# lenskit/csr

Hardware: AMD Instinct MI355X
Metric: spmv_gflops (higher is better)
Workload: dtype f64

## Files before the change

### csr_amd/csrc/spmv.hip

```cpp
#include "spmv_plan.h"

#include <algorithm>
#include <ctime>

namespace csrk {
template <bool R32>
__device__ __forceinline__ double spmv_prod(double a, double x)
{
    const double t = a * x;
    return R32 ? (double)(float)t : t;
}

void free_spmv_plan(SpmvPlan *p) { delete p; }

void spmv_plan_bytes_by_part(const SpmvPlan *p, int64_t out[5])
{
    for (int i = 0; i < 5; i++) out[i] = 0;
    auto add = [&](int part, std::initializer_list<const DevBuf *> bufs) {
        for (const DevBuf *b : bufs) out[part] += (int64_t)b->bytes;
    };
    for (const AccPanel *ap : p->acc) add(0, {&ap->row_list, &ap->vals, &ap->idx, &ap->tile_row0, &ap->segs, &ap->wg_seg, &ap->partial, &ap->z});
    const Panel &t = p->tier1;
    add(1, {&t.row_list, &t.rp, &t.ci, &t.vs, &t.tile, &t.group, &t.carry_row, &t.carry_val, &t.y, &t.crp, &t.cidx});
    const LightStream *l = &p->ls;
    add(2, {&l->vals, &l->idx, &l->rowids, &l->tile_base, &l->carry_row, &l->carry_val});
    add(3, {&l->xg, &l->a_col, &l->a_dst, &l->blk_start, &l->round_start, &l->round_tile0, &l->wg_round0, &p->hot_slot, &p->hot_cols, &p->xh});
    add(4, {&p->tile_row, &p->carry_row, &p->carry_val, &p->rp_light, &p->cut_pos, &p->cut_cum, &p->tile_cut, &p->heavy_row, &p->seg_off,
            &p->seg_row, &p->seg_part, &p->xwide});
}

int64_t spmv_plan_bytes(const SpmvPlan *p)
{
    int64_t part[5];
    spmv_plan_bytes_by_part(p, part);
    return part[0] + part[1] + part[2] + part[3] + part[4];
}


template <int VT>
__device__ __forceinline__ void load_val_pair(const void *vs, int64_t k, bool two, double &v0, double &v1)
{
    if (VT == CSRK_VAL_F64) {
        const double *p = (const double *)vs + k;
        if (two) {
            f64x2_t t = __builtin_nontemporal_load((const F64x2 *)p);
            v0 = t.x;
            v1 = t.y;
        } else {
            v0 = *p;
            v1 = 0.0;
        }
    } else if (VT == CSRK_VAL_F32) {
        const float *p = (const float *)vs + k;
        if (two) {
// ... 349 lines not shown
        }
        __syncthreads();
        const int nlong = s_nlong;
        for (int q = wv; q < nlong; q += PT / WAVE) {
            int r = s_long[q];
            int s = r ? s_rend[r - 1] : 0;
            int e = s_rend[r];
            double acc = 0.0;
            for (int k = s + lane; k < e; k += WAVE) acc += s_prod[k];
            acc = wave_sum(acc);
            if (lane == 0) {
                if (r < nr) {
                    yp[i0 + r] = acc;
                } else {
                    *(pt.cslot >= 0 ? yp + pt.cslot : carry_val + t) = acc;
                }
            }
        }
        pt = nx;
    }
#undef PANEL_LOAD_TILE
}

typedef float f32x4_t __attribute__((ext_vector_type(4)));
template <class SV> struct AccVals;
template <> struct AccVals<double> {
    f64x2_t v[4];
    __device__ __forceinline__ void load(const double *tile, int lane)
    {
        const f64x2_t *vp = (const f64x2_t *)tile;
#pragma unroll
        for (int q = 0; q < 4; q++) v[q] = __builtin_nontemporal_load(vp + q * WAVE + lane);
    }
    __device__ __forceinline__ void get(double (&a)[ACC_K]) const
    {
#pragma unroll
        for (int q = 0; q < 4; q++) {
            a[2 * q] = v[q].x;
            a[2 * q + 1] = v[q].y;
        }
    }
};
template <> struct AccVals<float> {
    f32x4_t v[2];
    __device__ __forceinline__ void load(const float *tile, int lane)
    {
        const f32x4_t *vp = (const f32x4_t *)tile;
#pragma unroll
        for (int q = 0; q < 2; q++) v[q] = __builtin_nontemporal_load(vp + q * WAVE + lane);
    }
    __device__ __forceinline__ void get(double (&a)[ACC_K]) const
    {
#pragma unroll
        for (int q = 0; q < 2; q++) {
            a[4 * q] = (double)v[q].x;
            a[4 * q + 1] = (double)v[q].y;
            a[4 * q + 2] = (double)v[q].z;
            a[4 * q + 3] = (double)v[q].w;
        }
    }
};

template <int CB, int PT, bool R32 = false, class SV = double, class XT = double>
__global__ __launch_bounds__(PT) void spmv_acc_kernel(const SV *__restrict__ pvals, const uint16_t *__restrict__ pidx,
                                                     const int32_t *__restrict__ tile_row0,
                                                     const XT *__restrict__ x, int32_t ncols,
                                                     const AccSeg *__restrict__ segs, const int32_t *__restrict__ wg_seg,
                                                     int32_t H, double *__restrict__ partial)
{
    extern __shared__ __align__(16) unsigned char acc_smem[];
    double *s_x = (double *)acc_smem;
    double *s_acc = s_x + CB + 2;
    const int Hpad = (H + 1) & ~1;
    double *s_hval = s_acc + Hpad;
    int32_t *s_hrow = (int32_t *)(s_hval + ACC_SEG_TILES);
    constexpr int NW = PT / WAVE;
    const int tid = threadIdx.x, lane = tid & (WAVE - 1), wv = tid / WAVE;

    for (int h = tid; h < Hpad; h += PT) s_acc[h] = 0.0;
    if (tid < 2) s_x[CB + tid] = 0.0;
    const unsigned long long below = lane ? (~0ull >> (WAVE - lane)) : 0ull;
    const unsigned long long upto = below | (1ull << lane);

    int cur_blk = -1;
    const int sb = wg_seg[blockIdx.x], se = wg_seg[blockIdx.x + 1];
    for (int si = sb; si < se; si++) {
        const AccSeg sg = segs[si];
        if (sg.blk != cur_blk) {
            cur_blk = sg.blk;
            const int32_t w0 = sg.blk * CB;
            const int wlen = ncols - w0 < CB ? ncols - w0 : CB;
            if (wlen == CB) {
                constexpr int WL = CB / 2 / PT;
                f64x2_t v[WL];
#pragma unroll
                for (int u = 0; u < WL; u++) {
                    if (sizeof(XT) == 8) {
                        v[u] = *((const F64x2 *)(x + w0) + tid + u * PT);
                    } else {
                        const f32x2_t t = *((const F32x2 *)(x + w0) + tid + u * PT);
                        v[u].x = (double)t.x;
                        v[u].y = (double)t.y;
                    }
                }
#pragma unroll
                for (int u = 0; u < WL; u++) ((f64x2_t *)s_x)[tid + u * PT] = v[u];
            } else {
                for (int k = tid; k < wlen; k += PT) s_x[k] = (double)x[w0 + k];
            }
        }
        __syncthreads();

        const int nt = sg.ntiles;
        AccVals<SV> v, vn;
        u32x4_t ix, ixn;
        int32_t tr0 = 0, tr0n = 0;
        int t = wv;
        const int64_t pstep = (int64_t)gridDim.x;
        if (t < nt) {
            const u32x4_t *ip = (const u32x4_t *)(pidx + (sg.ptile0 + t * pstep) * ACC_TILE);
            v.load(pvals + (sg.ptile0 + t * pstep) * ACC_TILE, lane);
            ix = __builtin_nontemporal_load(ip + lane);
            tr0 = tile_row0[sg.tile0 + t];
        }
        for (; t < nt; t += NW) {
            const bool more = t + NW < nt;
            if (more) {
                const u32x4_t *ip = (const u32x4_t *)(pidx + (sg.ptile0 + (t + NW) * pstep) * ACC_TILE);
                vn.load(pvals + (sg.ptile0 + (t + NW) * pstep) * ACC_TILE, lane);
                ixn = __builtin_nontemporal_load(ip + lane);
                tr0n = tile_row0[sg.tile0 + t + NW];
            }
            const uint32_t e[ACC_K] = {ix.x & 0xffffu, ix.x >> 16, ix.y & 0xffffu, ix.y >> 16,
                                       ix.z & 0xffffu, ix.z >> 16, ix.w & 0xffffu, ix.w >> 16};
            double a[ACC_K];
            v.get(a);
            double xv[ACC_K];
#pragma unroll
            for (int j = 0; j < ACC_K; j++) xv[j] = s_x[e[j] & ACC_COL_MASK];
            int rw[ACC_K];
            {
                int lsum = 0;
#pragma unroll
                for (int j = 0; j < ACC_K; j++) lsum += (int)(e[j] >> ACC_ROW_SHIFT);
                int run = tr0 + wave_exscan_i32(lsum, lane);
#pragma unroll
                for (int j = 0; j < ACC_K; j++) {
                    run += (int)(e[j] >> ACC_ROW_SHIFT);
                    rw[j] = run;
                }
            }
            const int hr = rw[0];
            int cur = hr;
            double acc = 0.0, hs = 0.0;
            bool nb = false;
#pragma unroll
            for (int j = 0; j < ACC_K; j++) {
                const int r = rw[j];
                if (r != cur) {
                    if (!nb) {
                        hs = acc;
                        nb = true;
                    } else {
                        atomicAdd(&s_acc[cur], acc);
                    }
                    acc = 0.0;
                    cur = r;
                }
                if (R32) acc += spmv_prod<true>(a[j], xv[j]);
                else acc += a[j] * xv[j];
            }
            const int tr = cur;
            const double ts = acc;
            if (!nb) hs = acc;
            const int tr_prev = wave_up1_i32(tr, -1);
            const bool ne = lane > 0 && tr_prev != hr;
            const double T = wave_segscan(ts, nb || ne, lane);
            const double T_prev = wave_up1_f64(T, 0.0);
// ... 197 lines not shown
        tb = __builtin_amdgcn_readfirstlane(tile_base[t]);
    }
    for (int64_t R = R_begin; R < R_end; R += R_step) {
    if (RND) {
        __syncthreads();
#pragma unroll
        for (int q = 0; q < RQ; q++) ((f64x2_t *)s_rnd)[q * LS_THREADS + threadIdx.x] = rv[q];
        __syncthreads();
        if (R + R_step < R_end) round_request(R + R_step);
    }
    const int64_t rt1 = round_t1(R);
    for (t = round_t0(R) + wv; t < rt1; t += NW) {
        int64_t t_next = t + NW;
        if (t_next >= rt1) {
            t_next = t;
            if (R + R_step < R_end) {
                const int64_t tf = round_t0(R + R_step) + wv;
                if (tf < round_t1(R + R_step)) t_next = tf;
            }
        }
        uint32_t e[ACC_K];
        if constexpr (I24) {
            const uint32_t lo[4] = {ix[0].x, ix[0].y, ix[0].z, ix[0].w}, hi[2] = {ix[1].x, ix[1].y};
#pragma unroll
            for (int j = 0; j < ACC_K; j++)
                e[j] = __builtin_amdgcn_perm(hi[j >> 2], lo[j >> 1],
                                             0x0c000000u | ((4u + (j & 3)) << 16) | ((2u * (j & 1) + 1u) << 8) | (2u * (j & 1)));
        } else {
            const uint32_t w[ACC_K] = {ix[0].x, ix[0].y, ix[0].z, ix[0].w, ix[1].x, ix[1].y, ix[1].z, ix[1].w};
#pragma unroll
            for (int j = 0; j < ACC_K; j++) e[j] = w[j];
        }
        double a[ACC_K];
        v.get(a);
        double gv[ACC_K], lv[ACC_K];
        bool inl[ACC_K];
        if (RND) {
#pragma unroll
            for (int j = 0; j < ACC_K; j++) {
                const uint32_t c = e[j] & COL_MASK;
                const bool hot = (e[j] & HOT_BIT) != 0;
                inl[j] = c != PAD && (!hot || (int32_t)c < n_lds);
                gv[j] = 0.0;
                if (hot && (int32_t)c >= n_lds) gv[j] = xh[c];
            }
        } else {
#pragma unroll
            for (int j = 0; j < ACC_K; j++) {
                const uint32_t c = e[j] & LS_COL_MASK;
                const bool hot = (e[j] & LS_HOT_BIT) != 0;
                inl[j] = hot && (int32_t)c < n_lds;
                gv[j] = 0.0;
                const double *g = hot ? xh + c : x + c;
                if (!inl[j] && c != LS_PAD) gv[j] = *g;
            }
        }
        int32_t rid[LS_RID];
#pragma unroll
        for (int i = 0; i < LS_RID; i++) {
            const int run = tb - 1 + lane + i * WAVE;
            const int runc = run < 0 ? 0 : (run > n_runs - 1 ? n_runs - 1 : run);
            rid[i] = DENSE ? runc : rowids[runc];
        }
        asm volatile("" ::: "memory");
        {
            const int64_t tn = t_next;
            idx_request(ixn, tn);
// ... 238 lines not shown
                dn[q] = k < k1 ? __builtin_nontemporal_load(a_dst + k) : 0;
            }
        }
#pragma unroll
        for (int q = 0; q < LS_STAGE_IPT; q++)
            if (c[q] >= 0) xg[d[q]] = s_x[c[q]];
        if (kn < k1) {
#pragma unroll
            for (int q = 0; q < LS_STAGE_IPT; q++) c[q] = cn[q], d[q] = dn[q];
        }
    }
}

int spmv_kernel_attributes()
{
    for (const void *f : {(const void *)spmv_acc_kernel<ACC_CB, ACC_THREADS>, (const void *)spmv_lstream_kernel<LS_PLAIN>,
                          (const void *)spmv_lstream_kernel<LS_RND>, (const void *)spmv_lstream_kernel<LS_PLAIN, true>,
                          (const void *)spmv_lstream_kernel<LS_RND, true>, (const void *)spmv_acc_kernel<ACC_CB, ACC_THREADS, true>,
                          (const void *)spmv_lstream_kernel<LS_PLAIN, false, true>, (const void *)spmv_lstream_kernel<LS_RND, false, true>,
                          (const void *)spmv_lstream_kernel<LS_PLAIN, true, true>, (const void *)spmv_lstream_kernel<LS_RND, true, true>,
                          (const void *)spmv_acc_kernel<ACC_CB, ACC_THREADS, false, float>,
                          (const void *)spmv_acc_kernel<ACC_CB, ACC_THREADS, true, float>,
                          (const void *)spmv_lstream_kernel<LS_PLAIN, false, false, float>, (const void *)spmv_lstream_kernel<LS_RND, false, false, float>,
                          (const void *)spmv_lstream_kernel<LS_PLAIN, true, false, float>, (const void *)spmv_lstream_kernel<LS_RND, true, false, float>,
                          (const void *)spmv_lstream_kernel<LS_PLAIN, false, true, float>, (const void *)spmv_lstream_kernel<LS_RND, false, true, float>,
                          (const void *)spmv_lstream_kernel<LS_PLAIN, true, true, float>, (const void *)spmv_lstream_kernel<LS_RND, true, true, float>,
                          (const void *)spmv_lstream_kernel<LS_RND24>, (const void *)spmv_lstream_kernel<LS_RND24, true>,
                          (const void *)spmv_lstream_kernel<LS_RND24, false, true>, (const void *)spmv_lstream_kernel<LS_RND24, true, true>,
                          (const void *)spmv_lstream_kernel<LS_RND24, false, false, float>, (const void *)spmv_lstream_kernel<LS_RND24, true, false, float>,
                          (const void *)spmv_lstream_kernel<LS_RND24, false, true, float>, (const void *)spmv_lstream_kernel<LS_RND24, true, true, float>,
                          (const void *)spmv_acc_kernel<ACC_CB, ACC_THREADS, false, double, float>,
                          (const void *)spmv_acc_kernel<ACC_CB, ACC_THREADS, true, double, float>,
                          (const void *)spmv_acc_kernel<ACC_CB, ACC_THREADS, false, float, float>,
                          (const void *)spmv_acc_kernel<ACC_CB, ACC_THREADS, true, float, float>})
        CSRK_HIP(hipFuncSetAttribute(f, hipFuncAttributeMaxDynamicSharedMemorySize, (int)(160 * 1024)));
    CSRK_HIP(hipFuncSetAttribute((const void *)ls_stage_kernel<double>, hipFuncAttributeMaxDynamicSharedMemorySize, (int)(LS_STAGE_WMAX * 8)));
    CSRK_HIP(hipFuncSetAttribute((const void *)ls_stage_kernel<float>, hipFuncAttributeMaxDynamicSharedMemorySize, (int)(LS_STAGE_WMAX * 8)));
    return CSRK_OK;
}

static int get_plan_locked(Matrix *m, hipStream_t s, SpmvPlan **out, bool launching)
{
    if (launching) m->spmv_calls++;
    const char *env = getenv("CSRK_SPMV_HEAVY_SPLIT"), *env_hot = getenv("CSRK_SPMV_HOT"), *env_ls = getenv("CSRK_SPMV_STREAM");
    const bool eager = (env && env[0] == '1') || (env_hot && env_hot[0] == '1') || (env_ls && env_ls[0] == '1') || !launching;
    const bool want_split = eager || m->spmv_calls >= 2;
    if (m->spmv_plan && !m->spmv_plan->split_considered && want_split && m->spmv_plan->algo == CSRK_SPMV_MERGE &&
        !m->spmv_plan->profiling) {
        if (hipDeviceSynchronize() != hipSuccess) {
            set_error("device synchronisation failed: %s", hipGetErrorString(hipGetLastError()));
            return CSRK_ERR_HIP;
        }
        free_spmv_plan(m->spmv_plan);
        m->spmv_plan = nullptr;
    }
    if (!m->spmv_plan) {
        SpmvPlan *p = new (std::nothrow) SpmvPlan();
        CSRK_REQUIRE(p, "out of host memory");
        p->algo = m->spmv_algo == CSRK_SPMV_AUTO ? CSRK_SPMV_MERGE : m->spmv_algo;
        (void)s;
        int rc = build_spmv_plan(m, p, want_split);
        if (rc == CSRK_OK && hipDeviceSynchronize() != hipSuccess) {
            set_error("SpMV plan construction failed: %s", hipGetErrorString(hipGetLastError()));
            rc = CSRK_ERR_HIP;
        }
        if (rc != CSRK_OK) {
            delete p;
// ... 58 lines not shown
            J.row_list = rows;
            J.H = H;
            J.n_wg = n_wg;
            J.G = G;
            J.extra = extra;
            J.crp = crp;
            J.cidx = cidx;
            J.cval = cval;
            epi.j[epi.n++] = J;
            return CSRK_OK;
        };
        if (do_light && p->ls.on && p->ls.n_cold) {
            KernelTimer ks(p, s, 3);
            const unsigned gs = (unsigned)(ceil_div(p->ls.n_stage_blk, 8) * 8);
            ls_stage_kernel<XT><<<gs, LS_STAGE_THREADS, (size_t)p->ls.stage_w * 8, s>>>(
                d_x, m->ncols, p->ls.stage_w, p->ls.a_col.as<uint16_t>(), p->ls.a_dst.as<int32_t>(),
                p->ls.blk_start.as<int32_t>(), p->ls.n_stage_blk, p->ls.xg.as<double>());
            ks.stop();
            CSRK_LAUNCH_CHECK();
        }
        if (do_light && p->n_hot && !(p->ls.on && p->ls.n_cold)) {
            hot_pack_kernel<XT><<<(unsigned)ceil_div(p->n_hot, 256), 256, 0, s>>>(d_x, p->hot_cols.as<int32_t>(), p->n_hot,
                                                                            p->xh.as<double>());
            CSRK_LAUNCH_CHECK();
        }
        bool t0_rides = false;
        if (do_heavy && p->n_heavy && !p->acc.empty()) {
            KernelTimer kh(p, s, 1);
            for (AccPanel *ap : p->acc) {
                if (ap->f32)
                    spmv_acc_kernel<ACC_CB, ACC_THREADS, R32, float, XT><<<(unsigned)ap->n_wg, ACC_THREADS, ap->lds, s>>>(
                        ap->vals.as<float>(), ap->idx.as<uint16_t>(), ap->tile_row0.as<int32_t>(), d_x, m->ncols,
                        ap->segs.as<AccSeg>(), ap->wg_seg.as<int32_t>(), ap->nrow, ap->partial.as<double>());
                else
                    spmv_acc_kernel<ACC_CB, ACC_THREADS, R32, double, XT><<<(unsigned)ap->n_wg, ACC_THREADS, ap->lds, s>>>(
                        ap->vals.as<double>(), ap->idx.as<uint16_t>(), ap->tile_row0.as<int32_t>(), d_x, m->ncols,
                        ap->segs.as<AccSeg>(), ap->wg_seg.as<int32_t>(), ap->nrow, ap->partial.as<double>());
                CSRK_LAUNCH_CHECK();
            }
            kh.stop();
        }
        if (do_heavy && p->n_heavy && p->tier1.on) {
            Panel *pn = &p->tier1;
            KernelTimer kh(p, s, 2);
#define PANEL_ARGS(PP)                                                                                              \
    pn->rp.as<PP>(), pn->ci.as<int32_t>(), pn->vs.as<double>(), d_x, m->ncols, pn->y.as<double>(),                    \
        pn->tile.as<PanelTile>(), pn->group.as<PanelGroup>(), pn->rows, pn->carry_row.as<int32_t>(),                  \
        pn->carry_val.as<double>(), pn->nnz, pn->cb, rider
            PanelRider rider = {pn->groups, nullptr, nullptr, 0, 0};
            if (PANEL_T1 / WAVE == 4 && do_heavy && p->acc.size() == 1 && p->acc[0]->z.p) {
                AccPanel *ap = p->acc[0];
                rider.partial = ap->partial.as<double>();
                rider.z = ap->z.as<double>();
                rider.H = ap->nrow;
                rider.n_wg = ap->n_wg;
                t0_rides = true;
            }
            const unsigned grid = (unsigned)(pn->groups + (t0_rides ? ceil_div(rider.H, WAVE) : 0));
            if (pn->p64) spmv_panel_kernel<int64_t, PANEL_T1, R32, XT><<<grid, PANEL_T1, 0, s>>>(PANEL_ARGS(int64_t));
            else spmv_panel_kernel<int32_t, PANEL_T1, R32, XT><<<grid, PANEL_T1, 0, s>>>(PANEL_ARGS(int32_t));
#undef PANEL_ARGS
            kh.stop();
            CSRK_LAUNCH_CHECK();
        }
        if (do_light) {
#define MERGE_ARGS_LIGHT(CI)                                                                                        \
// ... 401 lines not shown
    for (int c = 0; c < 4; c++) mean_ms[c] = cnt[c] ? (float)(tot[c] / cnt[c]) : 0.f;
    p->ev_used = 0;
    return CSRK_OK;
}

int csrk_spmv_profile_end(csrk_handle_t h, int *n_records, float *mean_ms)
{
    float ms4[4] = {0.f, 0.f, 0.f, 0.f};
    CSRK_REQUIRE(n_records && mean_ms, "output is NULL");
    CSRK_TRY(csrk_spmv_profile_end4(h, n_records, ms4));
    for (int c = 0; c < 3; c++) mean_ms[c] = ms4[c];
    return CSRK_OK;
}

int csrk_spmv_plan_stats(csrk_handle_t h, int64_t *out, int n)
{
    Matrix *m = from_handle(h);
    if (!m) return CSRK_ERR_INVALID;
    CSRK_REQUIRE(out && n >= 0, "out is NULL");
    SpmvPlan *p = nullptr;
    CSRK_TRY(get_plan(m, nullptr, &p));
    const Panel &t1 = p->tier1;
    int64_t a_tiles = 0, a_rows = 0, a_nnz = 0, a_nb = 0;
    for (const AccPanel *ap : p->acc) {
        a_tiles += ap->tiles;
        a_rows += ap->nrow;
        a_nnz += ap->nnz;
        a_nb = ap->nb;
    }
    const bool af = !p->acc.empty();
    const int64_t plan_bytes = spmv_plan_bytes(p);
    int64_t part[5];
    spmv_plan_bytes_by_part(p, part);
    const int64_t v[34] = {p->algo == CSRK_SPMV_MERGE ? p->n_tiles : p->n_segs,
                           p->algo == CSRK_SPMV_MERGE ? p->tile_items : VEC_SEG,
                           p->n_heavy, p->algo == CSRK_SPMV_MERGE ? p->nnz_light : m->nnz,
                           a_tiles, a_nb, p->heavy_min, af ? ACC_CB : 0, p->n_heavy ? 2 : 0, a_rows, a_nnz,
                           t1.nrow, t1.rows, t1.nnz, p->tier1_min, t1.cb,
                           p->n_hot, (int64_t)(p->hot_cover * 1e6), af ? 1 : 0, p->hot_slots,
                           p->ls.on ? 1 : 0, p->ls.n_tiles, p->ls.n_runs, p->ls.grid, p->ls.n_cold, plan_bytes,
                           p->ls.round_start.p ? p->ls.stage_tiles : 0,
                           af ? (int64_t)p->acc[0]->n_wg : 0, 0, part[0], part[1], part[2], part[3], part[4]};
    for (int i = 0; i < n && i < 34; i++) out[i] = v[i];
    return CSRK_OK;
}


int csrk_spmv_plan_info(csrk_handle_t h, int64_t *n_tiles, int32_t *tile_items)
{
    Matrix *m = from_handle(h);
    if (!m) return CSRK_ERR_INVALID;
    SpmvPlan *p = nullptr;
    CSRK_TRY(get_plan(m, nullptr, &p));
    if (n_tiles) *n_tiles = p->algo == CSRK_SPMV_MERGE ? p->n_tiles : p->n_segs;
    if (tile_items) *tile_items = p->algo == CSRK_SPMV_MERGE ? p->tile_items : VEC_SEG;
    return CSRK_OK;
}

}
```

### csr_amd/csrc/spmv_plan.h

```cpp
#pragma once
#include "common.h"
#include "wave.h"

#include <vector>

namespace csrk {

template <int VT> struct ValLoad;
template <> struct ValLoad<CSRK_VAL_F64> {
    static __device__ __forceinline__ double at(const void *v, int64_t k) { return ((const double *)v)[k]; }
};
template <> struct ValLoad<CSRK_VAL_F32> {
    static __device__ __forceinline__ double at(const void *v, int64_t k) { return (double)((const float *)v)[k]; }
};
template <> struct ValLoad<CSRK_VAL_NONE> {
    static __device__ __forceinline__ double at(const void *, int64_t) { return 1.0; }
};

__device__ __forceinline__ double wave_sum(double v)
{
#pragma unroll
    for (int off = WAVE / 2; off > 0; off >>= 1) v += __shfl_down(v, off, WAVE);
    return v;
}
// ... 7 lines not shown
        acc += a;
        acc += b;
        acc += c;
        acc += d;
    }
    for (; k < e; k++) acc += p[k];
    return acc;
}

struct Panel {
    bool on = false, p64 = false;
    int32_t cb = 0, nb = 0, nrow = 0;
    int64_t rows = 0, tiles = 0, nnz = 0, groups = 0;
    DevBuf row_list;
    DevBuf rp, ci, vs, tile, group, carry_row, carry_val, y;
    int32_t ncs = 0;
    DevBuf crp, cidx;
};

struct AccSeg {
    int64_t tile0;
    int64_t ptile0;
    int32_t ntiles;
    int32_t blk;
};

struct AccPanel {
    int32_t nrow = 0, nb = 0, n_wg = 0;
    int64_t tiles = 0, nnz = 0, n_segs = 0;
    size_t lds = 0;
    DevBuf row_list, vals, idx, tile_row0, segs, wg_seg, partial;
    DevBuf z;
    bool f32 = false;
};

struct LightStream {
    bool on = false;
    int64_t n_tiles = 0;
    int32_t n_runs = 0, n_out = 0;
    unsigned grid = 0;
    DevBuf vals, idx, rowids, tile_base, carry_row, carry_val;
    bool idx24 = false;
    bool f32 = false;
    bool dense = false;
    int64_t n_cold = 0;
    int32_t n_stage_blk = 0, stage_w = 0;
    DevBuf xg, a_col, a_dst, blk_start;
    int32_t stage_tiles = 0;
    DevBuf round_start, round_tile0, wg_round0;
};

struct SpmvPlan {
    int algo = CSRK_SPMV_MERGE;
    int tile_items = 0;
    int64_t n_tiles = 0;
    DevBuf tile_row;
    DevBuf carry_row;
    DevBuf carry_val;
    bool split_considered = false;
    int32_t n_heavy = 0;
    int32_t heavy_min = 0;
    int32_t tier1_min = 0;
    int64_t nnz_light = 0;
    DevBuf rp_light;
    DevBuf cut_pos;
    DevBuf cut_cum;
// ... 93 lines not shown
    int64_t t0;
    int32_t nt;
    int32_t blk;
};
constexpr int ACC_CB = 4096;
constexpr int ACC_K = 8;
constexpr int ACC_TILE = WAVE * ACC_K;
constexpr int ACC_MAXROWS = 15936;
constexpr int ACC_FLOOR = 128;
constexpr int ACC_SEG_TILES = 256;
constexpr int ACC_THREADS = 1024;
constexpr int ACC_ROW_SHIFT = 13;
constexpr uint32_t ACC_COL_MASK = (1u << ACC_ROW_SHIFT) - 1;
constexpr int ACC_MAXSTEP = 7;

typedef uint32_t u32x4_t __attribute__((ext_vector_type(4)));
typedef uint32_t u32x2_t __attribute__((ext_vector_type(2)));

__host__ __device__ __forceinline__ int acc_val_slot(int e)
{
    const int lane = e >> 3, j = e & 7;
    return (j >> 1) * (2 * WAVE) + lane * 2 + (j & 1);
}
__host__ __device__ __forceinline__ int acc_idx_slot(int e)
{
    const int lane = e >> 3, j = e & 7;
    return (j >> 2) * (4 * WAVE) + lane * 4 + (j & 3);
}
template <class SV> __host__ __device__ __forceinline__ int acc_slot_of(int e)
{
    return sizeof(SV) == 8 ? acc_val_slot(e) : acc_idx_slot(e);
}

#ifndef CSRK_LS_THREADS
#define CSRK_LS_THREADS 512
#endif
constexpr int LS_THREADS = CSRK_LS_THREADS;
#ifndef CSRK_LS_HOT_LDS
#define CSRK_LS_HOT_LDS 15360
#endif
constexpr int LS_HOT_LDS = CSRK_LS_HOT_LDS;
#ifndef CSRK_LS_RND_CAP
#define CSRK_LS_RND_CAP 8192
#endif
constexpr int LS_RND_CAP = CSRK_LS_RND_CAP, LS_RND_MAXTILES = 128;
constexpr int LS_RND_HOT = (160 * 1024 - (CSRK_LS_THREADS / 64) * (512 + 2) * 8) / 8 - LS_RND_CAP;
constexpr int LS_RID = 4;
#ifndef CSRK_LS_SEQ
#define CSRK_LS_SEQ 3
#endif
constexpr int LS_SEQ = CSRK_LS_SEQ;
constexpr uint32_t LS_HOT_BIT = 1u << 31, LS_START_BIT = 1u << 30, LS_COL_MASK = (1u << 30) - 1;
constexpr uint32_t LS_PAD = LS_COL_MASK;
#ifndef CSRK_LS_IDX24
#define CSRK_LS_IDX24 1
#endif
constexpr uint32_t LS24_HOT_BIT = 1u << 23, LS24_COL_MASK = (1u << 22) - 1;
constexpr int LS24_START_SHIFT = 22;
constexpr int64_t LS24_TILE_BYTES = 512 * 3;

constexpr int VEC_SEG = 4096;


#ifndef CSRK_STAGE_TILES
#define CSRK_STAGE_TILES 8
#endif
// ... 11 lines not shown
```

### csr_amd/csrc/spmv_plan.hip

```cpp
#include "spmv_plan.h"

#include <algorithm>
#include <cstring>
#include <ctime>

namespace csrk {
struct PlanTrace {
    bool on;
    double t0;
    static double now()
    {
        timespec ts;
        clock_gettime(CLOCK_MONOTONIC, &ts);
        return ts.tv_sec * 1e3 + ts.tv_nsec * 1e-6;
    }
    PlanTrace() : on(getenv("CSRK_PLAN_TRACE") != nullptr), t0(0.0)
    {
        if (on) {
            (void)hipDeviceSynchronize();
            t0 = now();
        }
    }
    void lap(const char *what)
    {
// ... 552 lines not shown
        const int64_t L = L0 + d;
        const int64_t t = L / ACC_TILE;
        const int el = (int)(L % ACC_TILE);
        const int64_t pt = acc_phys_tile(t, wg_t0, n_wg);
        if (at < npad_p) {
            pvals[pt * ACC_TILE + acc_slot_of<SV>(el)] = (SV)0.0;
            pidx[pt * ACC_TILE + el] = (uint16_t)((uint32_t)cb | ((el ? (uint32_t)ACC_MAXSTEP : 0u) << ACC_ROW_SHIFT));
            if (el == 0) tile_row0[t] = c0 + p - g_p + ACC_MAXSTEP * (at + 1);
        } else {
            const int64_t k = lo_p + (at - npad_p);
            const uint32_t step_in = at == npad_p ? (uint32_t)(g_p - ACC_MAXSTEP * npad_p) : 0u;
            pvals[pt * ACC_TILE + acc_slot_of<SV>(el)] = (SV)ValLoad<VT>::at(vs, k);
            pidx[pt * ACC_TILE + el] = (uint16_t)((uint32_t)(ci[k] - b * cb) | ((el ? step_in : 0u) << ACC_ROW_SHIFT));
            if (el == 0) tile_row0[t] = c0 + p;
        }
    }
}

template <class SV>
__global__ __launch_bounds__(256) void acc_pad_kernel(const int64_t *__restrict__ off, int32_t n_heavy, int32_t n_blocks,
                                                     const int64_t *__restrict__ blk_tile0, SV *__restrict__ pvals,
                                                     uint16_t *__restrict__ pidx, const int64_t *__restrict__ wg_t0, int32_t n_wg)
{
    const int32_t b = blockIdx.x;
    if (b >= n_blocks) return;
    const int64_t cnt = off[(int64_t)(b + 1) * n_heavy] - off[(int64_t)b * n_heavy];
    const int64_t L0 = blk_tile0[b] * ACC_TILE + cnt, L1 = blk_tile0[b + 1] * ACC_TILE;
    for (int64_t L = L0 + threadIdx.x; L < L1; L += blockDim.x) {
        const int64_t pt = acc_phys_tile(L / ACC_TILE, wg_t0, n_wg);
        const int el = (int)(L % ACC_TILE);
        pvals[pt * ACC_TILE + acc_slot_of<SV>(el)] = (SV)0.0;
        pidx[pt * ACC_TILE + el] = (uint16_t)ACC_CB;
    }
}


template <class P>
__device__ __forceinline__ int32_t ls_row_of(const P *__restrict__ rpv, int32_t nrows, int64_t L)
{
    int32_t lo = 0, hi = nrows - 1;
    while (lo < hi) {
        const int32_t mid = lo + ((hi - lo) >> 1);
        if ((int64_t)rpv[mid + 1] > L)
            hi = mid;
        else
            lo = mid + 1;
    }
    return lo;
}

template <class P>
__global__ void ls_tilerow_kernel(const P *__restrict__ rpv, int32_t nrows, int64_t n_ent, int64_t n_tiles, int32_t *__restrict__ tile_row)
{
    const int64_t t = (int64_t)blockIdx.x * blockDim.x + threadIdx.x;
    if (t > n_tiles) return;
    const int64_t e0 = t * ACC_TILE;
    tile_row[t] = t < n_tiles && e0 < n_ent ? ls_row_of(rpv, nrows, e0) : nrows - 1;
}

template <class P>
__global__ void ls_rowflag_kernel(const P *__restrict__ rpv, int32_t nrows, int32_t *__restrict__ flag)
{
    const int64_t r = (int64_t)blockIdx.x * blockDim.x + threadIdx.x;
    if (r <= nrows) flag[r] = (r < nrows && rpv[r + 1] > rpv[r]) ? 1 : 0;
}

// ... 270 lines not shown
    int cus = 0;
    CSRK_HIP(hipDeviceGetAttribute(&cus, hipDeviceAttributeMultiprocessorCount, m->device));
    int64_t n_wg = cus > 0 ? cus : 256;
    if (n_wg > n_tiles) n_wg = n_tiles;
    if (n_wg < 1) n_wg = 1;
    std::vector<int64_t> wg_t0((size_t)n_wg + 1);
    int64_t share_max = 0;
    for (int64_t w = 0; w <= n_wg; w++) wg_t0[(size_t)w] = n_tiles * w / n_wg;
    for (int64_t w = 0; w < n_wg; w++) share_max = std::max(share_max, wg_t0[(size_t)w + 1] - wg_t0[(size_t)w]);
    const int64_t n_phys = share_max * n_wg;
    DevBuf d_wg_t0;
    CSRK_TRY(d_wg_t0.alloc((size_t)(n_wg + 1) * 8));
    CSRK_TRY(stage_h2d(d_wg_t0.p, wg_t0.data(), (size_t)(n_wg + 1) * 8, s));
    ap->f32 = VT == CSRK_VAL_F32;
    CSRK_TRY(ap->vals.alloc((size_t)n_phys * ACC_TILE * (ap->f32 ? 4 : 8)));
    CSRK_TRY(ap->idx.alloc((size_t)n_phys * ACC_TILE * 2));
    CSRK_TRY(ap->tile_row0.alloc((size_t)(n_tiles ? n_tiles : 1) * 4));
    const int32_t fill_waves = (int32_t)ceil_div(n, WAVE);
#define ACC_FILL(SV)                                                                                                   \
    do {                                                                                                               \
        acc_fill_kernel<P, VT, SV><<<(unsigned)ceil_div((int64_t)nb * fill_waves * WAVE, 256), 256, 0, s>>>(           \
            rp, m->d_colinds, m->d_values, ap->row_list.as<int32_t>(), n, nb, ACC_CB, off.as<int64_t>(),               \
            bends.as<int64_t>(), pstart.as<int32_t>(), gap.as<int32_t>(), ap->vals.as<SV>(), ap->idx.as<uint16_t>(),   \
            ap->tile_row0.as<int32_t>(), d_wg_t0.as<int64_t>(), (int32_t)n_wg, fill_waves);                            \
        CSRK_LAUNCH_CHECK();                                                                                           \
        acc_pad_kernel<SV><<<(unsigned)nb, 256, 0, s>>>(off.as<int64_t>(), n, nb, bends.as<int64_t>(), ap->vals.as<SV>(), \
                                                        ap->idx.as<uint16_t>(), d_wg_t0.as<int64_t>(), (int32_t)n_wg); \
        CSRK_LAUNCH_CHECK();                                                                                           \
    } while (0)
    if (ap->f32) ACC_FILL(float);
    else ACC_FILL(double);
#undef ACC_FILL
    tr.lap("  tier 0: fill");
    std::vector<AccSeg> segs;
    std::vector<int32_t> wg_seg((size_t)n_wg + 1);
    int32_t b = 0;
    for (int64_t w = 0; w < n_wg; w++) {
        wg_seg[(size_t)w] = (int32_t)segs.size();
        int64_t t = wg_t0[(size_t)w];
        const int64_t t_end = wg_t0[(size_t)w + 1];
        while (t < t_end) {
            while (t0[b + 1] <= t) b++;
            int64_t e = t_end < t0[b + 1] ? t_end : t0[b + 1];
            if (e - t > ACC_SEG_TILES) e = t + ACC_SEG_TILES;
            AccSeg sg;
            sg.tile0 = t;
            sg.ptile0 = (t - wg_t0[(size_t)w]) * n_wg + w;
            sg.ntiles = (int32_t)(e - t);
            sg.blk = b;
            segs.push_back(sg);
            t = e;
        }
    }
    wg_seg[(size_t)n_wg] = (int32_t)segs.size();
    CSRK_TRY(ap->segs.alloc(segs.size() * sizeof(AccSeg)));
    CSRK_TRY(ap->wg_seg.alloc(wg_seg.size() * 4));
    CSRK_TRY(stage_h2d(ap->segs.p, segs.data(), segs.size() * sizeof(AccSeg), s));
    CSRK_TRY(stage_h2d(ap->wg_seg.p, wg_seg.data(), wg_seg.size() * 4, s));
    CSRK_TRY(ap->partial.alloc((size_t)n_wg * n * 8));
    CSRK_TRY(ap->z.alloc((size_t)n * 8));
    ap->lds = (size_t)(ACC_CB + 2) * 8 + (size_t)((n + 1) & ~1) * 8 + (size_t)ACC_SEG_TILES * 12;
    CSRK_TRY(spmv_kernel_attributes());
    CSRK_HIP(hipStreamSynchronize(s));
    ap->nrow = n;
    ap->nb = nb;
    ap->n_wg = (int32_t)n_wg;
// ... 788 lines not shown
```

Measured before the change: 783.0.

## Compress heavy-tier f64 values into lossless 57-bit shared-exponent planes

Adds a plan-time pass that checks each accumulator tile's exponent range and re-encodes eligible tiles into a packed plane format. Each value keeps its 32 low bits, 16 middle mantissa bits, a 4-bit exponent delta plus 4 mantissa bits, and a sign bit, using 57 bits per value instead of 64. Tiles that cannot be encoded this way spill their high halves to a side raw buffer. The spmv accumulator kernel decodes these values back to exact doubles, which cuts the value bytes streamed per nonzero in a bandwidth-bound kernel at the cost of extra integer ALU work and a uniform branch. It also adds a waitcnt before the main loop and census statistics.

```diff
diff --git a/csr_amd/csrc/spmv.hip b/csr_amd/csrc/spmv.hip
--- a/csr_amd/csrc/spmv.hip
+++ b/csr_amd/csrc/spmv.hip
@@ -19,7 +19,7 @@
     auto add = [&](int part, std::initializer_list<const DevBuf *> bufs) {
         for (const DevBuf *b : bufs) out[part] += (int64_t)b->bytes;
     };
-    for (const AccPanel *ap : p->acc) add(0, {&ap->row_list, &ap->vals, &ap->idx, &ap->tile_row0, &ap->segs, &ap->wg_seg, &ap->partial, &ap->z});
+    for (const AccPanel *ap : p->acc) add(0, {&ap->row_list, &ap->vals, &ap->raw_hi, &ap->idx, &ap->tile_row0, &ap->segs, &ap->wg_seg, &ap->partial, &ap->z});
     const Panel &t = p->tier1;
     add(1, {&t.row_list, &t.rp, &t.ci, &t.vs, &t.tile, &t.group, &t.carry_row, &t.carry_val, &t.y, &t.crp, &t.cidx});
     const LightStream *l = &p->ls;
@@ -435,7 +435,7 @@
 #pragma unroll
         for (int q = 0; q < 4; q++) v[q] = __builtin_nontemporal_load(vp + q * WAVE + lane);
     }
-    __device__ __forceinline__ void get(double (&a)[ACC_K]) const
+    __device__ __forceinline__ void get(double (&a)[ACC_K], int32_t, const uint16_t *, int) const
     {
 #pragma unroll
         for (int q = 0; q < 4; q++) {
@@ -443,6 +443,7 @@
             a[2 * q + 1] = v[q].y;
         }
     }
+    static __device__ __forceinline__ const double *tile(const double *vals, int64_t pt) { return vals + pt * ACC_TILE; }
 };
 template <> struct AccVals<float> {
     f32x4_t v[2];
@@ -452,7 +453,7 @@
 #pragma unroll
         for (int q = 0; q < 2; q++) v[q] = __builtin_nontemporal_load(vp + q * WAVE + lane);
     }
-    __device__ __forceinline__ void get(double (&a)[ACC_K]) const
+    __device__ __forceinline__ void get(double (&a)[ACC_K], int32_t, const uint16_t *, int) const
     {
 #pragma unroll
         for (int q = 0; q < 2; q++) {
@@ -462,6 +463,57 @@
             a[4 * q + 3] = (double)v[q].w;
         }
     }
+    static __device__ __forceinline__ const float *tile(const float *vals, int64_t pt) { return vals + pt * ACC_TILE; }
+};
+template <> struct AccVals<P57Tile> {
+    u32x4_t p0[2], p1;
+    u32x2_t p2;
+    uint32_t p3;
+    __device__ __forceinline__ void load(const P57Tile *tile, int lane)
+    {
+        const unsigned char *b = tile->b;
+        p0[0] = __builtin_nontemporal_load((const u32x4_t *)(b + P57_P0) + lane);
+        p0[1] = __builtin_nontemporal_load((const u32x4_t *)(b + P57_P0) + WAVE + lane);
+        p1 = __builtin_nontemporal_load((const u32x4_t *)(b + P57_P1) + lane);
+        p2 = __builtin_nontemporal_load((const u32x2_t *)(b + P57_P2) + lane);
+        p3 = __builtin_nontemporal_load(b + P57_P3 + lane);
+    }
+    template <bool Z> __device__ __forceinline__ void decode(uint32_t w, uint32_t (&hi)[ACC_K]) const
+    {
+        const uint32_t eb = (((w >> P57_META_SHIFT) & 0x7ffu) - (uint32_t)P57_ZERO) << 4;
+        const uint32_t f[2] = {p2.x ^ 0xf0f0f0f0u, p2.y ^ 0xf0f0f0f0u};
+        const uint32_t pw[4] = {p1.x, p1.y, p1.z, p1.w};
+#pragma unroll
+        for (int j = 0; j < ACC_K; j++) {
+            const uint32_t t = (f[j >> 2] >> (8 * (j & 3))) & 0xffu;
+            const uint32_t ts = t | ((p3 << (15 - j)) & 0x8000u);
+            uint32_t top = ts + eb;
+            if (Z) top = t ? top : ts;
+            hi[j] = (j & 1) ? __builtin_amdgcn_alignbit(top, pw[j >> 1], 16) : __builtin_amdgcn_perm(top, pw[j >> 1], 0x05040100u);
+        }
+    }
+    __device__ __forceinline__ void get(double (&a)[ACC_K], int32_t word, const uint16_t *raw_hi, int lane) const
+    {
+        const uint32_t lo[ACC_K] = {p0[0].x, p0[0].y, p0[0].z, p0[0].w, p0[1].x, p0[1].y, p0[1].z, p0[1].w};
+        const uint32_t w = (uint32_t)__builtin_amdgcn_readfirstlane(word);
+        uint32_t hi[ACC_K];
+        if (w & (uint32_t)P57_RAW_BIT) {
+            const uint32_t m32[ACC_K] = {p1.x & 0xffffu, p1.x >> 16, p1.y & 0xffffu, p1.y >> 16,
+                                         p1.z & 0xffffu, p1.z >> 16, p1.w & 0xffffu, p1.w >> 16};
+            const u32x4_t h = ((const u32x4_t *)raw_hi)[(int64_t)(w >> P57_META_SHIFT) * WAVE + lane];
+            const uint32_t h16[ACC_K] = {h.x << 16, h.x & 0xffff0000u, h.y << 16, h.y & 0xffff0000u,
+                                         h.z << 16, h.z & 0xffff0000u, h.w << 16, h.w & 0xffff0000u};
+#pragma unroll
+            for (int j = 0; j < ACC_K; j++) hi[j] = h16[j] | m32[j];
+        } else if (w & (uint32_t)P57_HASZERO_BIT) {
+            decode<true>(w, hi);
+        } else {
+            decode<false>(w, hi);
+        }
+#pragma unroll
+        for (int j = 0; j < ACC_K; j++) a[j] = __hiloint2double((int)hi[j], (int)lo[j]);
+    }
+    static __device__ __forceinline__ const P57Tile *tile(const P57Tile *vals, int64_t pt) { return vals + pt; }
 };
 
 template <int CB, int PT, bool R32 = false, class SV = double, class XT = double>
@@ -469,8 +521,10 @@
                                                      const int32_t *__restrict__ tile_row0,
                                                      const XT *__restrict__ x, int32_t ncols,
                                                      const AccSeg *__restrict__ segs, const int32_t *__restrict__ wg_seg,
-                                                     int32_t H, double *__restrict__ partial)
-{
+                                                     int32_t H, double *__restrict__ partial,
+                                                     const uint16_t *__restrict__ raw_hi = nullptr)
+{
+    constexpr bool P57 = sizeof(SV) == sizeof(P57Tile);
     extern __shared__ __align__(16) unsigned char acc_smem[];
     double *s_x = (double *)acc_smem;
     double *s_acc = s_x + CB + 2;
@@ -522,22 +576,23 @@
         const int64_t pstep = (int64_t)gridDim.x;
         if (t < nt) {
             const u32x4_t *ip = (const u32x4_t *)(pidx + (sg.ptile0 + t * pstep) * ACC_TILE);
-            v.load(pvals + (sg.ptile0 + t * pstep) * ACC_TILE, lane);
+            v.load(AccVals<SV>::tile(pvals, sg.ptile0 + t * pstep), lane);
             ix = __builtin_nontemporal_load(ip + lane);
             tr0 = tile_row0[sg.tile0 + t];
         }
+        __builtin_amdgcn_s_waitcnt(0x0f70);
         for (; t < nt; t += NW) {
             const bool more = t + NW < nt;
             if (more) {
                 const u32x4_t *ip = (const u32x4_t *)(pidx + (sg.ptile0 + (t + NW) * pstep) * ACC_TILE);
-                vn.load(pvals + (sg.ptile0 + (t + NW) * pstep) * ACC_TILE, lane);
+                vn.load(AccVals<SV>::tile(pvals, sg.ptile0 + (t + NW) * pstep), lane);
                 ixn = __builtin_nontemporal_load(ip + lane);
                 tr0n = tile_row0[sg.tile0 + t + NW];
             }
             const uint32_t e[ACC_K] = {ix.x & 0xffffu, ix.x >> 16, ix.y & 0xffffu, ix.y >> 16,
                                        ix.z & 0xffffu, ix.z >> 16, ix.w & 0xffffu, ix.w >> 16};
             double a[ACC_K];
-            v.get(a);
+            v.get(a, tr0, raw_hi, lane);
             double xv[ACC_K];
 #pragma unroll
             for (int j = 0; j < ACC_K; j++) xv[j] = s_x[e[j] & ACC_COL_MASK];
@@ -546,7 +601,7 @@
                 int lsum = 0;
 #pragma unroll
                 for (int j = 0; j < ACC_K; j++) lsum += (int)(e[j] >> ACC_ROW_SHIFT);
-                int run = tr0 + wave_exscan_i32(lsum, lane);
+                int run = (P57 ? tr0 & P57_ROW_MASK : tr0) + wave_exscan_i32(lsum, lane);
 #pragma unroll
                 for (int j = 0; j < ACC_K; j++) {
                     run += (int)(e[j] >> ACC_ROW_SHIFT);
@@ -810,7 +865,7 @@
             for (int j = 0; j < ACC_K; j++) e[j] = w[j];
         }
         double a[ACC_K];
-        v.get(a);
+        v.get(a, 0, nullptr, lane);
         double gv[ACC_K], lv[ACC_K];
         bool inl[ACC_K];
         if (RND) {
@@ -1115,7 +1170,11 @@
                           (const void *)spmv_acc_kernel<ACC_CB, ACC_THREADS, false, double, float>,
                           (const void *)spmv_acc_kernel<ACC_CB, ACC_THREADS, true, double, float>,
                           (const void *)spmv_acc_kernel<ACC_CB, ACC_THREADS, false, float, float>,
-                          (const void *)spmv_acc_kernel<ACC_CB, ACC_THREADS, true, float, float>})
+                          (const void *)spmv_acc_kernel<ACC_CB, ACC_THREADS, true, float, float>,
+                          (const void *)spmv_acc_kernel<ACC_CB, ACC_THREADS, false, P57Tile>,
+                          (const void *)spmv_acc_kernel<ACC_CB, ACC_THREADS, true, P57Tile>,
+                          (const void *)spmv_acc_kernel<ACC_CB, ACC_THREADS, false, P57Tile, float>,
+                          (const void *)spmv_acc_kernel<ACC_CB, ACC_THREADS, true, P57Tile, float>})
         CSRK_HIP(hipFuncSetAttribute(f, hipFuncAttributeMaxDynamicSharedMemorySize, (int)(160 * 1024)));
     CSRK_HIP(hipFuncSetAttribute((const void *)ls_stage_kernel<double>, hipFuncAttributeMaxDynamicSharedMemorySize, (int)(LS_STAGE_WMAX * 8)));
     CSRK_HIP(hipFuncSetAttribute((const void *)ls_stage_kernel<float>, hipFuncAttributeMaxDynamicSharedMemorySize, (int)(LS_STAGE_WMAX * 8)));
@@ -1240,6 +1299,10 @@
                     spmv_acc_kernel<ACC_CB, ACC_THREADS, R32, float, XT><<<(unsigned)ap->n_wg, ACC_THREADS, ap->lds, s>>>(
                         ap->vals.as<float>(), ap->idx.as<uint16_t>(), ap->tile_row0.as<int32_t>(), d_x, m->ncols,
                         ap->segs.as<AccSeg>(), ap->wg_seg.as<int32_t>(), ap->nrow, ap->partial.as<double>());
+                else if (ap->p57)
+                    spmv_acc_kernel<ACC_CB, ACC_THREADS, R32, P57Tile, XT><<<(unsigned)ap->n_wg, ACC_THREADS, ap->lds, s>>>(
+                        ap->vals.as<P57Tile>(), ap->idx.as<uint16_t>(), ap->tile_row0.as<int32_t>(), d_x, m->ncols,
+                        ap->segs.as<AccSeg>(), ap->wg_seg.as<int32_t>(), ap->nrow, ap->partial.as<double>(), ap->raw_hi.as<uint16_t>());
                 else
                     spmv_acc_kernel<ACC_CB, ACC_THREADS, R32, double, XT><<<(unsigned)ap->n_wg, ACC_THREADS, ap->lds, s>>>(
                         ap->vals.as<double>(), ap->idx.as<uint16_t>(), ap->tile_row0.as<int32_t>(), d_x, m->ncols,
@@ -1707,7 +1770,14 @@
     const int64_t plan_bytes = spmv_plan_bytes(p);
     int64_t part[5];
     spmv_plan_bytes_by_part(p, part);
-    const int64_t v[34] = {p->algo == CSRK_SPMV_MERGE ? p->n_tiles : p->n_segs,
+    int64_t a_census = 0, a_raw = 0;
+    for (const AccPanel *ap : p->acc)
+        if (ap->n_raw >= 0) {
+            a_census += ap->tiles;
+            a_raw += ap->n_raw;
+        }
+    const int64_t a_fmt = !af ? 0 : (p->acc[0]->p57 ? 2 : (p->acc[0]->f32 ? 0 : 1));
+    const int64_t v[40] = {p->algo == CSRK_SPMV_MERGE ? p->n_tiles : p->n_segs,
                            p->algo == CSRK_SPMV_MERGE ? p->tile_items : VEC_SEG,
                            p->n_heavy, p->algo == CSRK_SPMV_MERGE ? p->nnz_light : m->nnz,
                            a_tiles, a_nb, p->heavy_min, af ? ACC_CB : 0, p->n_heavy ? 2 : 0, a_rows, a_nnz,
@@ -1715,8 +1785,9 @@
                            p->n_hot, (int64_t)(p->hot_cover * 1e6), af ? 1 : 0, p->hot_slots,
                            p->ls.on ? 1 : 0, p->ls.n_tiles, p->ls.n_runs, p->ls.grid, p->ls.n_cold, plan_bytes,
                            p->ls.round_start.p ? p->ls.stage_tiles : 0,
-                           af ? (int64_t)p->acc[0]->n_wg : 0, 0, part[0], part[1], part[2], part[3], part[4]};
-    for (int i = 0; i < n && i < 34; i++) out[i] = v[i];
+                           af ? (int64_t)p->acc[0]->n_wg : 0, 0, part[0], part[1], part[2], part[3], part[4],
+                           a_fmt, a_census, a_raw, p->ls.on && !p->ls.f32 ? 1 : 0, 0, 0};
+    for (int i = 0; i < n && i < 40; i++) out[i] = v[i];
     return CSRK_OK;
 }
 
diff --git a/csr_amd/csrc/spmv_plan.h b/csr_amd/csrc/spmv_plan.h
--- a/csr_amd/csrc/spmv_plan.h
+++ b/csr_amd/csrc/spmv_plan.h
@@ -63,6 +63,9 @@
     DevBuf row_list, vals, idx, tile_row0, segs, wg_seg, partial;
     DevBuf z;
     bool f32 = false;
+    bool p57 = false;
+    int64_t n_raw = -1;
+    DevBuf raw_hi;
 };
 
 struct LightStream {
@@ -222,6 +225,31 @@
     return sizeof(SV) == 8 ? acc_val_slot(e) : acc_idx_slot(e);
 }
 
+constexpr int P57_P0 = 0, P57_P1 = 2048, P57_P2 = 3072, P57_P3 = 3584;
+constexpr int64_t P57_TILE_BYTES = 3648;
+constexpr int P57_RAW_DENOM = 16;
+constexpr int P57_ZERO = 15;
+constexpr int P57_WORD_SHIFT = 14;
+constexpr int32_t P57_ROW_MASK = (1 << P57_WORD_SHIFT) - 1, P57_RAW_BIT = 1 << P57_WORD_SHIFT;
+constexpr int P57_META_SHIFT = P57_WORD_SHIFT + 1;
+constexpr uint32_t P57_HASZERO_BIT = 1u << (P57_META_SHIFT + 11);
+constexpr int64_t P57_MAX_RAW = 1ll << (32 - P57_META_SHIFT);
+struct P57Tile {
+    unsigned char b[P57_TILE_BYTES];
+};
+static_assert(ACC_MAXROWS <= (1 << P57_WORD_SHIFT), "a heavy-row index fits below the raw flag");
+static_assert(P57_TILE_BYTES % 16 == 0 && P57_P3 + WAVE == P57_TILE_BYTES, "four planes, 16-B aligned tiles");
+__host__ __device__ __forceinline__ int p57_p0_off(int e) { return P57_P0 + 4 * acc_idx_slot(e); }
+__host__ __device__ __forceinline__ int p57_p1_off(int e) { return P57_P1 + 2 * e; }
+__host__ __device__ __forceinline__ int p57_p2_off(int e) { return P57_P2 + e; }
+__host__ __device__ __forceinline__ int p57_p3_off(int e) { return P57_P3 + (e >> 3); }
+__host__ __device__ __forceinline__ int p57_exp_of(uint32_t hi) { return (int)((hi >> 20) & 0x7ffu); }
+__host__ __device__ __forceinline__ bool p57_odd_value(uint32_t hi, uint32_t lo)
+{
+    const int ex = p57_exp_of(hi);
+    return ex == 0x7ff || (ex == 0 && ((hi & 0xfffffu) | lo) != 0);
+}
+
 #ifndef CSRK_LS_THREADS
 #define CSRK_LS_THREADS 512
 #endif
diff --git a/csr_amd/csrc/spmv_plan.hip b/csr_amd/csrc/spmv_plan.hip
--- a/csr_amd/csrc/spmv_plan.hip
+++ b/csr_amd/csrc/spmv_plan.hip
@@ -608,6 +608,97 @@
         pvals[pt * ACC_TILE + acc_slot_of<SV>(el)] = (SV)0.0;
         pidx[pt * ACC_TILE + el] = (uint16_t)ACC_CB;
     }
+}
+
+__device__ __forceinline__ void p57_load_tile(const double *__restrict__ tile, int lane, uint32_t (&lo)[ACC_K], uint32_t (&hi)[ACC_K])
+{
+    const u32x4_t *vp = (const u32x4_t *)tile;
+#pragma unroll
+    for (int q = 0; q < 4; q++) {
+        const u32x4_t v = vp[q * WAVE + lane];
+        lo[2 * q] = v.x;
+        hi[2 * q] = v.y;
+        lo[2 * q + 1] = v.z;
+        hi[2 * q + 1] = v.w;
+    }
+}
+
+__global__ __launch_bounds__(256) void p57_census_kernel(const double *__restrict__ vals, int64_t n_tiles,
+                                                        const int64_t *__restrict__ wg_t0, int32_t n_wg, int32_t *__restrict__ census)
+{
+    const int64_t t = ((int64_t)blockIdx.x * blockDim.x + threadIdx.x) / WAVE;
+    const int lane = threadIdx.x & (WAVE - 1);
+    if (t >= n_tiles) return;
+    uint32_t lo[ACC_K], hi[ACC_K];
+    p57_load_tile(vals + acc_phys_tile(t, wg_t0, n_wg) * ACC_TILE, lane, lo, hi);
+    int emax = 0, emin = 0x7ff, odd = 0, zero = 0;
+#pragma unroll
+    for (int j = 0; j < ACC_K; j++) {
+        const int ex = p57_exp_of(hi[j]);
+        odd |= p57_odd_value(hi[j], lo[j]) ? 1 : 0;
+        zero |= ((hi[j] & 0x7fffffffu) | lo[j]) == 0 ? 1 : 0;
+        if (ex > 0 && ex < 0x7ff) {
+            emax = ex > emax ? ex : emax;
+            emin = ex < emin ? ex : emin;
+        }
+    }
+#pragma unroll
+    for (int d = WAVE / 2; d > 0; d >>= 1) {
+        emax = max(emax, __shfl_xor(emax, d, WAVE));
+        emin = min(emin, __shfl_xor(emin, d, WAVE));
+        odd |= __shfl_xor(odd, d, WAVE);
+        zero |= __shfl_xor(zero, d, WAVE);
+    }
+    const bool raw = odd || (emax > 0 && emax - emin >= P57_ZERO);
+    if (lane == 0) census[t] = emax | (raw ? 1 << 11 : 0) | (zero ? 1 << 12 : 0);
+}
+
+__global__ __launch_bounds__(256) void p57_convert_kernel(const double *__restrict__ vals, int64_t n_tiles,
+                                                         const int64_t *__restrict__ wg_t0, int32_t n_wg,
+                                                         const int32_t *__restrict__ words, P57Tile *__restrict__ out,
+                                                         uint16_t *__restrict__ raw_hi, int32_t *__restrict__ tile_row0)
+{
+    const int64_t t = ((int64_t)blockIdx.x * blockDim.x + threadIdx.x) / WAVE;
+    const int lane = threadIdx.x & (WAVE - 1);
+    if (t >= n_tiles) return;
+    const int64_t pt = acc_phys_tile(t, wg_t0, n_wg);
+    uint32_t lo[ACC_K], hi[ACC_K];
+    p57_load_tile(vals + pt * ACC_TILE, lane, lo, hi);
+    const uint32_t w = (uint32_t)words[t];
+    const bool raw = (w & (uint32_t)P57_RAW_BIT) != 0;
+    unsigned char *b = out[pt].b;
+    u32x4_t q0 = {lo[0], lo[1], lo[2], lo[3]}, q1 = {lo[4], lo[5], lo[6], lo[7]};
+    ((u32x4_t *)(b + P57_P0))[lane] = q0;
+    ((u32x4_t *)(b + P57_P0))[WAVE + lane] = q1;
+    u32x4_t m;
+    m.x = (hi[0] & 0xffffu) | (hi[1] << 16);
+    m.y = (hi[2] & 0xffffu) | (hi[3] << 16);
+    m.z = (hi[4] & 0xffffu) | (hi[5] << 16);
+    m.w = (hi[6] & 0xffffu) | (hi[7] << 16);
+    ((u32x4_t *)(b + P57_P1))[lane] = m;
+    u32x2_t p2 = {0u, 0u};
+    uint32_t p3 = 0;
+    if (raw) {
+        u32x4_t h;
+        h.x = (hi[0] >> 16) | (hi[1] & 0xffff0000u);
+        h.y = (hi[2] >> 16) | (hi[3] & 0xffff0000u);
+        h.z = (hi[4] >> 16) | (hi[5] & 0xffff0000u);
+        h.w = (hi[6] >> 16) | (hi[7] & 0xffff0000u);
+        ((u32x4_t *)raw_hi)[(int64_t)(w >> P57_META_SHIFT) * WAVE + lane] = h;
+    } else {
+        const int E = (int)((w >> P57_META_SHIFT) & 0x7ffu);
+#pragma unroll
+        for (int j = 0; j < ACC_K; j++) {
+            const bool zero = ((hi[j] & 0x7fffffffu) | lo[j]) == 0;
+            const uint32_t byte = zero ? (uint32_t)P57_ZERO << 4 : ((uint32_t)(E - p57_exp_of(hi[j])) << 4) | ((hi[j] >> 16) & 0xfu);
+            if (j < 4) p2.x |= byte << (8 * j);
+            else p2.y |= byte << (8 * (j - 4));
+            p3 |= (hi[j] >> 31) << j;
+        }
+    }
+    ((u32x2_t *)(b + P57_P2))[lane] = p2;
+    b[P57_P3 + lane] = (unsigned char)p3;
+    if (lane == 0) tile_row0[t] |= (int32_t)w;
 }
 
 
@@ -944,6 +1035,40 @@
     else ACC_FILL(double);
 #undef ACC_FILL
     tr.lap("  tier 0: fill");
+    const char *env57 = getenv("CSRK_SPMV_P57");
+    if (!ap->f32 && n_tiles > 0 && !(env57 && env57[0] == '0')) {
+        DevBuf words;
+        CSRK_TRY(words.alloc((size_t)n_tiles * 4));
+        const unsigned g57 = (unsigned)ceil_div(n_tiles * WAVE, 256);
+        p57_census_kernel<<<g57, 256, 0, s>>>(ap->vals.as<double>(), n_tiles, d_wg_t0.as<int64_t>(), (int32_t)n_wg, words.as<int32_t>());
+        CSRK_LAUNCH_CHECK();
+        std::vector<int32_t> hw((size_t)n_tiles);
+        CSRK_TRY(stage_d2h(hw.data(), words.p, (size_t)n_tiles * 4, s));
+        int64_t n_raw = 0;
+        for (int64_t t = 0; t < n_tiles; t++) {
+            int32_t &w = hw[(size_t)t];
+            const bool raw = ((w >> 11) & 1) != 0;
+            w = raw ? P57_RAW_BIT | (int32_t)((uint32_t)n_raw << P57_META_SHIFT)
+                    : (int32_t)(((uint32_t)(w & 0x7ff) << P57_META_SHIFT) | ((w >> 12) & 1 ? P57_HASZERO_BIT : 0u));
+            n_raw += raw ? 1 : 0;
+        }
+        ap->n_raw = n_raw;
+        const bool want = (env57 && env57[0] == '1') || n_raw * P57_RAW_DENOM <= n_tiles;
+        if (want && n_raw <= P57_MAX_RAW) {
+            DevBuf planes;
+            CSRK_TRY(planes.alloc((size_t)n_phys * P57_TILE_BYTES));
+            CSRK_TRY(ap->raw_hi.alloc((size_t)n_raw * ACC_TILE * 2));
+            CSRK_TRY(stage_h2d(words.p, hw.data(), (size_t)n_tiles * 4, s));
+            p57_convert_kernel<<<g57, 256, 0, s>>>(ap->vals.as<double>(), n_tiles, d_wg_t0.as<int64_t>(), (int32_t)n_wg,
+                                                  words.as<int32_t>(), planes.as<P57Tile>(), ap->raw_hi.as<uint16_t>(),
+                                                  ap->tile_row0.as<int32_t>());
+            CSRK_LAUNCH_CHECK();
+            std::swap(ap->vals.p, planes.p);
+            std::swap(ap->vals.bytes, planes.bytes);
+            ap->p57 = true;
+        }
+        tr.lap("  tier 0: p57 census, planes");
+    }
     std::vector<AccSeg> segs;
     std::vector<int32_t> wg_seg((size_t)n_wg + 1);
     int32_t b = 0;
```

Result: no change. 777.4 (-0.7%).
